# abbomarengo/ml-trainer

Measured on AMD Instinct MI355X. Metric: samples/sec/node, higher is better.
Workload: dtype bf16; 1 GPU; model=src/model.py MLModel (default LeNet-5, 62,006 params), global_batch=32, per_gpu_batch=32, parallelism=dp1, optimizer=sgd lr=1e-3 momentum=0.9, hipgraph_steps=47, graph_prewarm=1, update=in-step, dp_transport=none, loss_finite=True

## Files before the change

ml_trainer_amd/csrc/bindings.cpp:

```cpp
#include <ATen/ATen.h>
#include <c10/hip/HIPStream.h>
#include <pybind11/pybind11.h>
#include <pybind11/stl.h>
#include <torch/extension.h>

#include <cmath>
#include <map>
#include <memory>

#include "mlt_kernels.h"
#include "mlt_comm.h"
#include "mlt_runtime.h"

namespace py = pybind11;
using at::Tensor;

namespace mlt {

hipStream_t cur_stream() { return c10::hip::getCurrentHIPStream().stream(); }

#define CHECK_CUDA_T(t) TORCH_CHECK((t).is_cuda(), #t " must be a device tensor")
#define CHECK_CONTIG(t) TORCH_CHECK((t).is_contiguous(), #t " must be contiguous")
#define CHECK_F32(t) TORCH_CHECK((t).scalar_type() == at::kFloat, #t " must be float32")

// ... 1202 lines not shown
    P_.slab1 = fp("slab1", B * C1 * 640);
    P_.i1 = get("i1", at::kByte, B * C1 * 196).data_ptr<uint8_t>();
    P_.i2 = get("i2", at::kByte, B * FLAT).data_ptr<uint8_t>();
    P_.targets = get("targets", at::kLong, B).data_ptr<int64_t>();
    P_.stats = get("stats", at::kDouble, 2).data_ptr<double>();
    P_.counters = reinterpret_cast<unsigned*>(get("counters", at::kInt, C1 + 1).data_ptr<int32_t>());
    P_.stage = bufs.contains("stage") ? get("stage", at::kByte, B * 3072).data_ptr<uint8_t>() : nullptr;
    P_.stage_meta = bufs.contains("stage_meta") ? get("stage_meta", at::kLong, B * 4).data_ptr<int64_t>() : nullptr;
    if (!P_.stage || !P_.stage_meta) P_.stage = nullptr, P_.stage_meta = nullptr;
    P_.cestat = bufs.contains("cestat") ? get("cestat", at::kDouble, B * 2).data_ptr<double>() : nullptr;
    P_.dtargets = nullptr;
    if (bufs.contains("stage2") && bufs.contains("meta2") && bufs.contains("metaN") && bufs.contains("stepinfo") &&
        bufs.contains("shadow") && bufs.contains("wimg")) {
      P_.stage2 = get("stage2", at::kByte, B * 3072).data_ptr<uint8_t>();
      P_.meta2 = get("meta2", at::kLong, B * 4).data_ptr<int64_t>();
      P_.metaN = get("metaN", at::kLong, B * 4).data_ptr<int64_t>();
      P_.stepinfo = get("stepinfo", at::kLong, 4).data_ptr<int64_t>();
      Tensor sh = bufs["shadow"].cast<Tensor>();
      check_dev(sh, "shadow", at::kShort, 1);
      keep_.push_back(sh);
      P_.shadow = reinterpret_cast<uint16_t*>(sh.data_ptr<int16_t>());
      shadow_n_ = sh.numel();
      P_.wimg = reinterpret_cast<uint16_t*>(get("wimg", at::kShort, lenet_mfma_wimg_elems()).data_ptr<int16_t>());
      TORCH_CHECK(P_.slab1 != nullptr && (int64_t)C1 * 640 >= lenet_mfma_slab_floats(cfg), "slab1 too small");
    }
    if (bufs.contains("trace")) P_.trace = get("trace", at::kFloat, 4096).data_ptr<float>();
    const char* pe = std::getenv("MLT_LENET_PREP");
    if (bufs.contains("prep") && bufs.contains("pmeta") && !(pe && std::string(pe) == "0")) {
      P_.prep = get("prep", at::kByte, B * 8192).data_ptr<uint8_t>();
      P_.pmeta = get("pmeta", at::kLong, B * 4).data_ptr<int64_t>();
    }
    const char* se = std::getenv("MLT_LENET_SPLIT");
    split_ = !(se && std::string(se) == "0");
    A_ = LeNetAug{};
    O_ = LeNetOpt{};
  }

  void set_aug(Tensor data, Tensor perm, Tensor ctrl, Tensor dtargets, int64_t seed, int pad, int flip,
               int batch_stride, std::vector<double> mean, std::vector<double> stdv) {
    A_ = make_aug(data, perm, ctrl, seed, pad, flip, batch_stride, mean, stdv);
    TORCH_CHECK(A_.ctrl != nullptr, "ctrl required");
    check_dev(dtargets, "dtargets", at::kLong, A_.n);
    P_.dtargets = dtargets.data_ptr<int64_t>();
    aug_keep_ = {data, perm, ctrl, dtargets};
    graphs_.clear();
  }

  void clear_aug() {
    A_.data = nullptr;
    P_.dtargets = nullptr;
    graphs_.clear();
  }

  void set_ctrl(Tensor ctrl) {
    check_dev(ctrl, "ctrl", at::kLong, 2, 8);
    A_.ctrl = ctrl.data_ptr<int64_t>();
    ctrl_keep_ = ctrl;
    graphs_.clear();
  }

  void set_opt(Tensor p, Tensor g, c10::optional<Tensor> s1, c10::optional<Tensor> s2, int kind, double lr,
               double momentum, double dampening, double wd, double beta1, double beta2, double eps,
               double lr_decay, double grad_scale, bool nesterov, bool maximize, c10::optional<Tensor> lr_t,
               bool lr_table, std::vector<int64_t> offsets) {
    const int64_t n = p.numel();
    check_dev(p, "p", at::kFloat, n);
// ... 51 lines not shown
    if (comm.is_none()) {
      comm_ = nullptr;
      comm_keep_ = py::none();
    } else {
      comm_ = &comm.cast<PyComm&>().raw();
      comm_keep_ = comm;
    }
    graphs_.clear();
  }

  void set_precision(int p) {
    TORCH_CHECK(p == 0 || p == 1, "precision: 0 (fp32) or 1 (bf16)");
    if (p == 1) TORCH_CHECK(P_.shadow && P_.wimg && P_.stage2 && P_.meta2 && P_.metaN && P_.stepinfo,
                            "bf16 engine buffers missing");
    prec_ = p;
    pack_ver_ = -1;
    graphs_.clear();
  }
  int precision() const { return prec_; }
  void set_fused_dp(bool f) {
    fused_dp_ = f;
    graphs_.clear();
  }
  bool fused_dp() const { return fused_dp_; }
  void set_split(bool s) {
    split_ = s;
    graphs_.clear();
  }
  bool split() const { return split_; }
  bool split_active(int B) const {
    if (prec_ != 1 || B <= 0 || B > max_b_) return false;
    return lenet_mfma_split_active(split_bits(LENET_FWD | LENET_CE | LENET_BWD), B, P_, A_);
  }
  int split_bits(int mode) const {
    return split_ || prec_ != 1 || !(mode & LENET_BWD) ? mode : mode | LENET_NOSPLIT;
  }

  void check_mode(int mode, int B) const {
    TORCH_CHECK(B > 0 && B <= max_b_, "batch ", B, " outside [1, ", max_b_, "]");
    if (prec_ == 1 && (mode & LENET_BWD)) {
      TORCH_CHECK((mode & LENET_FWD) && (mode & LENET_CE), "bf16 engine: training steps are FWD|CE|BWD");
      TORCH_CHECK(A_.ctrl != nullptr && O_.g != nullptr, "bf16 engine: set_ctrl / set_opt first");
      TORCH_CHECK(shadow_n_ >= O_.n, "bf16 engine: shadow smaller than the flat parameters");
    }
    TORCH_CHECK(!((mode & LENET_OPT) && (mode & LENET_REDUCE)),
                "LENET_OPT (fused local update) and LENET_REDUCE (all-reduce + update) are exclusive");
    if (mode & LENET_REDUCE) TORCH_CHECK(A_.ctrl != nullptr, "ctrl required for the data-parallel update");
    if (mode & (LENET_OPT | LENET_REDUCE)) TORCH_CHECK(O_.g != nullptr, "set_opt() first");
    if (mode & LENET_OPT) TORCH_CHECK(A_.ctrl != nullptr, "ctrl required for the fused optimizer");
    if ((mode & LENET_OPT) && O_.lr_table) TORCH_CHECK(A_.ctrl != nullptr, "lr table needs ctrl");
  }

  void run(int mode, int B) {
    check_mode(mode, B);
    const bool mf = prec_ == 1 && (mode & LENET_BWD);
    if (mf) launch_lenet_mfma_pack(cfg_, P_, O_, cur_stream());
    launch_step(cfg_, split_bits(mode), B, P_, A_, O_, comm_, xgmi_, cur_stream(), mf, fused_dp_);
  }

  void reduce_only(int B, bool exchange) {
    TORCH_CHECK(prec_ == 1 && P_.stepinfo && O_.g, "reduce_only: bf16 engine with set_opt");
    TORCH_CHECK(B > 0 && B <= max_b_, "reduce_only: batch");
    if (exchange) {
      TORCH_CHECK(xgmi_ != nullptr, "reduce_only: no xGMI transport");
      const XgmiFused X = xgmi_->fused_view();
      launch_lenet_mfma_reduce(cfg_, B, P_, O_, &X, cur_stream());
    } else {
      launch_lenet_mfma_reduce(cfg_, B, P_, O_, nullptr, cur_stream());
// ... 69 lines not shown
  void replay(int mode, int B, int nsteps) {
    auto it = graphs_.find(key(mode, B, nsteps));
    TORCH_CHECK(it != graphs_.end(), "no captured graph for this (mode, B, nsteps)");
    if (mode & LENET_BWD) sync_shadow();
    it->second->launch(cur_stream());
  }

  size_t graph_nodes(int mode, int B, int nsteps) const {
    auto it = graphs_.find(key(mode, B, nsteps));
    return it == graphs_.end() ? 0 : it->second->num_nodes();
  }

  void reset_graphs() { graphs_.clear(); }

 private:
  static int64_t key(int mode, int B, int nsteps) {
    return ((int64_t)mode << 48) | ((int64_t)B << 16) | (int64_t)nsteps;
  }
  int cfg_;
  int max_b_;
  LeNetPtrs P_{};
  LeNetAug A_{};
  LeNetOpt O_{};
  std::vector<Tensor> keep_, aug_keep_, opt_keep_;
  Tensor ctrl_keep_;
  Communicator* comm_ = nullptr;
  py::object comm_keep_ = py::none();
  XgmiAllReduce* xgmi_ = nullptr;
  py::object xgmi_keep_ = py::none();
  std::map<int64_t, std::unique_ptr<HipGraph>> graphs_;
  int prec_ = 0;
  bool fused_dp_ = true;
  bool split_ = true;
  int64_t shadow_n_ = 0;
  Tensor master_;
  int64_t pack_ver_ = -1;
};

}

PYBIND11_MODULE(TORCH_EXTENSION_NAME, m) {
  using namespace mlt;
  m.doc() = "ml_trainer_amd native gfx950 kernels and runtime";
  m.attr("ARCH") = "gfx950";
  m.def("flat_optim", &flat_optim, py::arg("p"), py::arg("g"), py::arg("s1"), py::arg("s2"), py::arg("kind"),
        py::arg("lr"), py::arg("momentum"), py::arg("dampening"), py::arg("weight_decay"), py::arg("beta1"),
        py::arg("beta2"), py::arg("eps"), py::arg("lr_decay"), py::arg("grad_scale"), py::arg("nesterov"),
        py::arg("maximize"), py::arg("lr_t") = py::none(), py::arg("lr_index") = py::none(),
        py::arg("step_t") = py::none(), py::arg("t_host") = 1.0, py::arg("shadow") = py::none(),
        py::arg("coef") = py::none());
  m.def("optim_chunk_elems", &optim_chunk_elems);
  m.def("flat_optim_seg", &flat_optim_seg, py::arg("p"), py::arg("g"), py::arg("s1"), py::arg("s2"),
        py::arg("chunks"), py::arg("wd"), py::arg("lr"), py::arg("beta1"), py::arg("beta2"), py::arg("eps"),
        py::arg("grad_scale"), py::arg("maximize"), py::arg("lr_t") = py::none(), py::arg("lr_index") = py::none(),
        py::arg("step_t") = py::none(), py::arg("t_host") = 1.0, py::arg("shadow") = py::none(),
        py::arg("coef") = py::none(), py::arg("skip") = py::none(), py::arg("max_blocks") = 0);
  m.def("lamb_step", &lamb_step, py::arg("p"), py::arg("g"), py::arg("m"), py::arg("v"), py::arg("chunks"),
        py::arg("tseg"), py::arg("wd"), py::arg("adapt"), py::arg("part"), py::arg("norms"), py::arg("trust"),
        py::arg("lr"), py::arg("beta1"), py::arg("beta2"), py::arg("eps"), py::arg("grad_scale"),
        py::arg("maximize"), py::arg("lr_t") = py::none(), py::arg("lr_index") = py::none(),
        py::arg("step_t") = py::none(), py::arg("t_host") = 1.0, py::arg("shadow") = py::none(),
        py::arg("coef") = py::none(), py::arg("skip") = py::none(), py::arg("max_blocks") = 0,
        py::arg("stages") = 7);
  m.def("sq_norm", &sq_norm);
  m.def("clip_coef", &clip_coef);
  m.def("cast_bf16", &cast_bf16);
// ... 99 lines not shown
      .def("async_error", &PyComm::async_error)
      .def("abort", &PyComm::abort);
  py::class_<PyXgmi>(m, "XgmiAllReduce", py::dynamic_attr())
      .def(py::init<int64_t, int, int, int, int>(), py::arg("capacity"), py::arg("world"), py::arg("rank"),
           py::arg("device"), py::arg("blocks") = 64)
      .def("handle", &PyXgmi::handle)
      .def("open", &PyXgmi::open)
      .def("all_reduce", &PyXgmi::all_reduce, py::arg("tensor"), py::arg("average") = true)
      .def("error", &PyXgmi::error)
      .def_property_readonly("world", [](PyXgmi& x) { return x.raw().world(); })
      .def_property("timeout_ms", &PyXgmi::timeout_ms, &PyXgmi::set_timeout_ms)
      .def_property("algo", &PyXgmi::algo, &PyXgmi::set_algo)
      .def_property("fault", &PyXgmi::fault, &PyXgmi::set_fault)
      .def_property("fused_two", &PyXgmi::fused_two, &PyXgmi::set_fused_two);
  py::class_<PyPrefetcher>(m, "PinnedPrefetcher")
      .def(py::init<int64_t, int, int>(), py::arg("slot_bytes"), py::arg("depth"), py::arg("device"))
      .def("slot", &PyPrefetcher::slot)
      .def("copy_to_device", &PyPrefetcher::copy_to_device)
      .def("acquire", &PyPrefetcher::acquire)
      .def("release", &PyPrefetcher::release)
      .def("ready", &PyPrefetcher::ready)
      .def("wait", &PyPrefetcher::wait)
      .def_property_readonly("depth", &PyPrefetcher::depth)
      .def_property_readonly("slot_bytes", &PyPrefetcher::slot_bytes);
  py::class_<LeNetEngine>(m, "LeNetEngine")
      .def(py::init<int, int, py::dict>())
      .def("set_aug", &LeNetEngine::set_aug)
      .def("set_comm", &LeNetEngine::set_comm)
      .def("set_xgmi", &LeNetEngine::set_xgmi)
      .def_property("fused_dp", &LeNetEngine::fused_dp, &LeNetEngine::set_fused_dp)
      .def("set_split", &LeNetEngine::set_split)
      .def("split", &LeNetEngine::split)
      .def("split_active", &LeNetEngine::split_active, py::arg("B"))
      .def("clear_aug", &LeNetEngine::clear_aug)
      .def("set_ctrl", &LeNetEngine::set_ctrl)
      .def("set_opt", &LeNetEngine::set_opt)
      .def("set_precision", &LeNetEngine::set_precision)
      .def("precision", &LeNetEngine::precision)
      .def("run", &LeNetEngine::run)
      .def("capture", &LeNetEngine::capture)
      .def("has_graph", &LeNetEngine::has_graph)
      .def("replay", &LeNetEngine::replay)
      .def("invalidate_shadow", &LeNetEngine::invalidate_shadow)
      .def("reduce_only", &LeNetEngine::reduce_only, py::arg("B"), py::arg("exchange"))
      .def("graph_nodes", &LeNetEngine::graph_nodes)
      .def("reset_graphs", &LeNetEngine::reset_graphs);
  m.attr("LENET_FWD") = (int)LENET_FWD;
  m.attr("LENET_CE") = (int)LENET_CE;
  m.attr("LENET_BWD") = (int)LENET_BWD;
  m.attr("LENET_OPT") = (int)LENET_OPT;
  m.attr("LENET_TRACE") = (int)LENET_TRACE;
  m.attr("LENET_REDUCE") = (int)LENET_REDUCE;
}
```

ml_trainer_amd/csrc/include/mlt_kernels.h:

```cpp
#pragma once
#include <hip/hip_runtime.h>
#include <stdint.h>

#include "mlt_optim.h"
#include "mlt_philox.h"

namespace mlt {

void launch_flat_optim(float* p, const float* g, float* s1, float* s2, int64_t n, const OptHyper& h,
                       const float* lr_ptr, const int64_t* lr_index_ptr, const int64_t* step_ptr, float t_host,
                       uint16_t* shadow_bf16, const float* coef_ptr, hipStream_t stream,
                       const unsigned* skip = nullptr);
int optim_chunk_elems();
void launch_flat_optim_seg(float* p, const float* g, float* s1, float* s2, int64_t n, const int* chunks,
                           int nchunks, const float* wd, int nt, const OptHyper& h, const float* lr_ptr,
                           const int64_t* lr_index_ptr, const int64_t* step_ptr, float t_host,
                           uint16_t* shadow_bf16, const float* coef_ptr, const unsigned* skip, int max_blocks,
                           hipStream_t stream);
void launch_lamb_step(float* p, const float* g, float* m, float* v, int64_t n, const int* chunks, int nchunks,
                      const int* tseg, const float* wd, const int* adapt, int nt, float* part, float* norms,
                      float* trust, const OptHyper& h, const float* lr_ptr, const int64_t* lr_index_ptr,
                      const int64_t* step_ptr, float t_host, uint16_t* shadow_bf16, const float* coef_ptr,
                      const unsigned* skip, int max_blocks, int stages, hipStream_t stream);
int sq_norm_partials_needed();
void launch_sq_norm(const float* x, int64_t n, float* part, float* out, hipStream_t stream);
void launch_clip_coef(const float* sq, float max_norm, float* coef, float* total_norm, hipStream_t stream);
void launch_cast_bf16(const float* x, uint16_t* y, int64_t n, hipStream_t stream);
void launch_transpose_bf16(const uint16_t* src, uint16_t* dst, int R, int C, hipStream_t stream);

enum LeNetCfg : int { LENET_DEFAULT = 0, LENET_TINY = 1 };
enum LeNetMode : int {
  LENET_FWD = 1,
  LENET_CE = 2,
  LENET_BWD = 4,
  LENET_OPT = 8,
  LENET_REDUCE = 16,
  LENET_TRACE = 256,
  LENET_STATS_DEFER = 16384,
  LENET_PROBE_NOF1T = 1 << 17,
  LENET_PROBE_NOF1W = 1 << 18,
  LENET_PROBE_NOF2 = 1 << 19,
  LENET_NOSPLIT = 1 << 20,
};

struct LeNetPtrs {
  const float *w1, *b1, *w2, *b2, *w3, *b3, *w4, *b4, *w5, *b5;
  float *gw1, *gb1, *gw2, *gb2, *gw3, *gb3, *gw4, *gb4, *gw5, *gb5;
  float *x, *p1, *p2, *h1, *h2, *logits, *dlogits, *dh2, *dh1, *dflat, *g1, *slab1;
  uint8_t *i1, *i2;
  int64_t* targets;
  const int64_t* dtargets;
  double* stats;
  unsigned* counters;
  uint8_t* stage;
  int64_t* stage_meta;
  double* cestat;
  uint8_t* stage2;
  int64_t* meta2;
  int64_t* metaN;
  int64_t* stepinfo;
  uint16_t* shadow;
  uint16_t* wimg;
  float* trace;
  uint8_t* prep;
  int64_t* pmeta;
};

struct LeNetAug {
  const uint8_t* data;
  int64_t step_host, sie_host;
  const int32_t* perm;
  int64_t* ctrl;
  int64_t n;
  int64_t perm_len;
  uint64_t seed;
  int pad;
  int flip;
  int batch_stride;
  float mean[3], std[3];
  float ascale[3], ashift[3];
};

struct LeNetOpt {
  float *p, *g, *s1, *s2;
  int64_t n;
  OptHyper h;
  const float* lr_ptr;
  int lr_table;
  int64_t off[10];
};

void launch_lenet(int cfg, int mode, int B, const LeNetPtrs& P, const LeNetAug& A, const LeNetOpt& O,
                  hipStream_t stream);
void launch_head_cls_fwd(const float* pooled, int B, int h, const float* wc, const float* bc, int L, float* logits,
                         hipStream_t st);
void launch_head_cls_bwd(const float* dlogits, const float* pooled, const float* wc, int B, int h, int L,
                         uint16_t* dpre, float* dwc, float* dbc, bool accumulate, hipStream_t st);
void launch_lenet_mfma(int cfg, int mode, int B, const LeNetPtrs& P, const LeNetAug& A, const LeNetOpt& O,
                       hipStream_t stream);
bool lenet_mfma_split_active(int mode, int B, const LeNetPtrs& P, const LeNetAug& A);
int lenet_mfma_slab_floats(int cfg);
int lenet_mfma_kw_blocks(int cfg);
void launch_lenet_mfma_apply(int cfg, const LeNetPtrs& P, const LeNetOpt& O, const unsigned* skip, hipStream_t stream);
struct XgmiFused;
void launch_lenet_mfma_dp(int cfg, int mode, int B, const LeNetPtrs& P, const LeNetAug& A, const LeNetOpt& O,
                          const XgmiFused& X, hipStream_t stream);
int lenet_mfma_wimg_elems();
bool lenet_mfma_trace_build();
void launch_lenet_mfma_reduce(int cfg, int B, const LeNetPtrs& P, const LeNetOpt& O, const XgmiFused* X,
                              hipStream_t stream);
int64_t lenet_mfma_xch_granules(int cfg);
void launch_lenet_mfma_pack(int cfg, const LeNetPtrs& P, const LeNetOpt& O, hipStream_t stream);

void launch_cifar_augment(const LeNetAug& A, int B, float* out, int64_t* targets_out, const int64_t* dtargets,
                          hipStream_t stream);

void launch_ce_fwd(const void* logits, bool bf16, const int64_t* tgt, int64_t B, int C, float* dl, float* acc,
                   float* correct, float* loss, int64_t ignore_index, float label_smoothing, hipStream_t st);
void launch_ce_bwd(const float* dl, const float* gout, const float* acc, int64_t n, void* out, bool bf16,
                   hipStream_t st);
void launch_accuracy(const void* logits, bool bf16, const int64_t* tgt, int64_t B, int C, float* out,
                     hipStream_t st);
int loss_partials_needed();
void launch_pointwise_loss_fwd(const float* p, const float* t, int64_t n, int mode, float* g, float* part,
                               float* out, hipStream_t st);
void launch_nll_fwd(const float* logp, const int64_t* tgt, int64_t B, int C, int64_t ignore_index, float* part,
                    float* out, hipStream_t st);
void launch_loss_scale_grad(const float* g, const float* gout, const float* stats, int64_t n, float* out,
                            hipStream_t st);
void launch_nll_bwd(const int64_t* tgt, int64_t B, int C, int64_t ignore_index, const float* gout,
                    const float* stats, float* out, hipStream_t st);
void launch_mcrmse(const float* p, const float* t, int64_t B, int C, float* col, float* out, hipStream_t st);

// ... 129 lines not shown
```

ml_trainer_amd/csrc/kernels/lenet_mfma.hip:

```cpp
#include "lenet_mfma.inc"

namespace mlt {
namespace lm {
void launch_ms(int cfg, int mode, int B, const LeNetPtrs& P, const LeNetAug& A, const LeNetOpt& O, hipStream_t st) {
  if (cfg == LENET_TINY)
    launch_ms_t<DmTiny>(mode, B, P, A, O, st);
  else
    launch_ms_t<DmDefault>(mode, B, P, A, O, st);
}
}

bool lenet_mfma_split_active(int mode, int B, const LeNetPtrs& P, const LeNetAug& A) {
  return lm::split_eligible(mode, B, P, A);
}

void launch_lenet_mfma_reduce(int cfg, int B, const LeNetPtrs& P, const LeNetOpt& O, const XgmiFused* X,
                              hipStream_t stream) {
  if (B <= 0) return;
  if (cfg == LENET_TINY)
    lm::reduce_only<lm::DmTiny>(cfg, B, P, O, X, stream);
  else
    lm::reduce_only<lm::DmDefault>(cfg, B, P, O, X, stream);
}
int lenet_mfma_slab_floats(int cfg) { return cfg == LENET_TINY ? lm::DmTiny::SLABN : lm::DmDefault::SLABN; }
int lenet_mfma_wimg_elems() { return lm::kWimgTot; }
bool lenet_mfma_trace_build() { return lm::kTraceBuild; }
int lenet_mfma_kw_blocks(int cfg) {
  return cfg == LENET_TINY ? lm::mw_conv_blocks<lm::DmTiny>() + lm::mw_fc_blocks<lm::DmTiny>() + 1
                           : lm::mw_conv_blocks<lm::DmDefault>() + lm::mw_fc_blocks<lm::DmDefault>() + 1;
}

void launch_lenet_mfma_apply(int cfg, const LeNetPtrs& P, const LeNetOpt& O, const unsigned* skip, hipStream_t stream) {
  if (O.n <= 0) return;
  const dim3 grid((unsigned)((O.n + 255) / 256));
  if (cfg == LENET_TINY)
    hipLaunchKernelGGL(lm::lenet_mapply<lm::DmTiny>, grid, dim3(256), 0, stream, P, O, skip);
  else
    hipLaunchKernelGGL(lm::lenet_mapply<lm::DmDefault>, grid, dim3(256), 0, stream, P, O, skip);
}

void launch_lenet_mfma_pack(int cfg, const LeNetPtrs& P, const LeNetOpt& O, hipStream_t stream) {
  if (cfg == LENET_TINY)
    lm::pack<lm::DmTiny>(P, O, stream);
  else
    lm::pack<lm::DmDefault>(P, O, stream);
}
// ... 12 lines not shown
```

ml_trainer_amd/csrc/kernels/lenet_mfma.inc:

```
#pragma once
#include <cstdlib>
#include <stdexcept>
#include <type_traits>

#include "mlt_common.h"
#include "mlt_kernels.h"
#include "mlt_optim.h"

namespace mlt {
namespace lm {

typedef __bf16 bf16x8 __attribute__((ext_vector_type(8)));
typedef float f32x4 __attribute__((ext_vector_type(4)));
typedef unsigned u32x4 __attribute__((ext_vector_type(4)));

__device__ __forceinline__ f32x4 mfma(u32x4 a, u32x4 b, f32x4 c) {
  return __builtin_amdgcn_mfma_f32_16x16x32_bf16(__builtin_bit_cast(bf16x8, a), __builtin_bit_cast(bf16x8, b), c, 0,
                                                 0, 0);
}

__device__ __forceinline__ void lbar() { asm volatile("s_waitcnt lgkmcnt(0)\n\ts_barrier" ::: "memory"); }

template <int KW>
__device__ __forceinline__ u32x4 fshift(u32x4 lo, u32x4 hi) {
// ... 48 lines not shown
  }
  if (e < kW2D) {
    const int q = e - kW2F, l = (q >> 3) & 63, j = q & 7, oc = l & 15, tap = 4 * (q >> 9) + (l >> 4);
    return (tap < 25 && oc < C2 && j < C1) ? off_w2 + (oc * C1 + j) * 25 + tap : -1;
  }
  const int q = e - kW2D, l = (q >> 3) & 63, j = q & 7, n = l & 15, gg = l >> 4;
  const int pp = 2 * (q >> 9) + (gg >> 1), oc = 8 * (gg & 1) + j, ic = n >> 1, kh = pp / 6;
  const int kw = pp - 6 * kh - 1 + (n & 1);
  (void)s;
  return (pp < 30 && ic < C1 && oc < C2 && kw >= 0 && kw < 5) ? off_w2 + (oc * C1 + ic) * 25 + kh * 5 + kw : -1;
}

template <int C1_, int C2_, int F1_, int F2_, int NC_>
struct Dm {
  static constexpr int C1 = C1_, C2 = C2_, F1 = F1_, F2 = F2_, NC = NC_, FLAT = C2_ * 25;
  static_assert(C1_ <= 8 && C2_ <= 16 && C2_ % 4 == 0 && F1_ % 4 == 0 && F2_ % 4 == 0 && NC_ <= 64, "dims");
  static constexpr int S1 = C1 * 76, S2OFF = (S1 + 3) & ~3, S2 = C2 * C1 * 25 + C2;
  static constexpr int SLABN = (S2OFF + S2 + 15) & ~15;
};
using DmDefault = Dm<6, 16, 120, 84, 10>;
using DmTiny = Dm<4, 8, 64, 32, 10>;

constexpr int kT = 1024;
constexpr int XCS = 48;
constexpr int P1CS = 32;
constexpr int XHS = 48;
constexpr int P1HS = 24;
constexpr int DCHS = 19;
constexpr int DCCS = 24;
constexpr int D1S = 28 * 32 + 16;
constexpr int kWgT = 256;
constexpr int kP13W = 7;
constexpr int kC1W = 8;
#ifndef MLT_LENET_TRACE_BUILD
#define MLT_LENET_TRACE_BUILD 0
#endif
constexpr bool kTraceBuild = MLT_LENET_TRACE_BUILD != 0;

constexpr int pow2_ge(int v) { return v <= 1 ? 1 : v <= 2 ? 2 : v <= 4 ? 4 : v <= 8 ? 8 : v <= 16 ? 16 : v <= 32 ? 32 : 64; }

template <int KS, int LD, int N, int K>
__device__ __forceinline__ void frag_rows(u32x4 (&f)[KS], const uint16_t* __restrict__ W, int tn) {
  const unsigned lane = threadIdx.x & 63;
  const unsigned row = min(16u * tn + (lane & 15), (unsigned)N - 1);
#pragma unroll
  for (int q = 0; q < KS; ++q) {
    const unsigned col = min(32u * q + 8 * (lane >> 4), (unsigned)((K - 1) / 8 * 8));
    f[q] = ld16(W, row * LD + col);
  }
}
template <int KS>
__device__ __forceinline__ float row_dot(const u32x4 (&f)[KS], const uint16_t* x) {
  const int g = (threadIdx.x & 63) >> 4;
  f32x4 acc = {0.f, 0.f, 0.f, 0.f};
#pragma unroll
  for (int q = 0; q < KS; ++q) acc = mfma(*reinterpret_cast<const u32x4*>(x + 32 * q + 8 * g), f[q], acc);
  return acc[0];
}

typedef short s16x4 __attribute__((ext_vector_type(4)));
typedef __attribute__((address_space(3))) s16x4 lds_s16x4;
template <int FLAT>
__device__ __forceinline__ int f1_chunk(int r, int c) {
  return r * (FLAT / 8 + 1) + (r & 1) + c;
}
template <int F1, int FLAT>
// ... 103 lines not shown
#pragma unroll
  for (int c = 0; c < 3; ++c) {
    const float u = in ? (float)img[(r * 32 + q) * 3 + c] : 0.f;
    v[c] = fmaf(u, A.ascale[c], A.ashift[c]);
  }
}

__device__ __forceinline__ int hmod(uint64_t h, unsigned span) {
  if (span == 9u) return (int)(h % 9u);
  const unsigned hi = (unsigned)(h >> 32) % span, lo = (unsigned)h % span;
  const unsigned r32 = (0xffffffffu % span + 1u) % span;
  return (int)((hi * r32 + lo) % span);
}

__device__ __forceinline__ void aug_params(const LeNetAug& A, int64_t step, int64_t pos, int& ci, int& cj, bool& fl) {
  const uint64_t h = mix64(mix64(A.seed + (uint64_t)step) ^ (uint64_t)pos);
  const unsigned span = 2 * A.pad + 1;
  ci = A.pad ? hmod(h, span) : 0;
  cj = A.pad ? hmod(h >> 20, span) : 0;
  fl = A.flip && ((h >> 40) & 1);
}

__device__ __forceinline__ void pool4(f32x4 a, float bias, float& pv, uint8_t& code) {
  float m = a[0];
  int k = 0;
  if (a[1] > m) { m = a[1]; k = 1; }
  if (a[2] > m) { m = a[2]; k = 2; }
  if (a[3] > m) { m = a[3]; k = 3; }
  m += bias;
  pv = m > 0.f ? m : 0.f;
  code = m > 0.f ? (uint8_t)k : (uint8_t)4;
}

template <class D, bool SPLIT>
__global__ __launch_bounds__(kT) void lenet_ms(uint8_t* __restrict__ pstage2, int64_t* __restrict__ pmeta2,
                                               const int64_t* __restrict__ pctrl, const uint16_t* __restrict__ pwimg,
                                               int64_t* __restrict__ pmetaN, int mode, float inv_B, LeNetPtrs P,
                                               LeNetAug A, LeNetOpt O, int B) {
  constexpr int C1 = D::C1, C2 = D::C2, FLAT = D::FLAT, F1 = D::F1, F2 = D::F2, NC = D::NC;
  using S = KsLds<D>;
  static_assert(offsetof(typename S::V::Fw, w2f) == offsetof(typename S::V::Fw, w1f) + 2 * kW2F,
                "forward fragment images must be contiguous");
  static_assert(sizeof(S) <= 160 * 1024, "LDS");
  __shared__ S L;
  const int bi = (int)blockIdx.x;
  const bool roleW = SPLIT && bi >= B;
  const bool doW = !SPLIT || roleW, doD = !SPLIT || !roleW;
  const int b = roleW ? bi - B : bi, t = threadIdx.x, lane = t & 63, g = lane >> 4, m = lane & 15;
  const int w = __builtin_amdgcn_readfirstlane(t >> 6);
  auto stamp = [&](int k) {
    if constexpr (!kTraceBuild) return;
    if (!(mode & LENET_TRACE)) return;
    lbar();
    __builtin_amdgcn_sched_barrier(0);
    unsigned long long c, wc;
    asm volatile("s_memtime %0\n\ts_memrealtime %1\n\ts_waitcnt lgkmcnt(0)" : "=s"(c), "=s"(wc)::"memory");
    __builtin_amdgcn_sched_barrier(0);
    if (t == 0) {
      L.tr[k] = c;
      if (k == 0) L.tr[14] = wc;
      if (k == 13) L.tr[15] = wc;
    }
  };
  if (kTraceBuild && (mode & LENET_TRACE) && t < 32) L.tr[t] = 0ull;
  if (kTraceBuild && (mode & LENET_TRACE) && t < 96) (&L.wtr[0][0])[t] = 0ull;
  auto wstamp = [&](int k) {
    if constexpr (!kTraceBuild) return;
    if (!(mode & LENET_TRACE)) return;
    __builtin_amdgcn_sched_barrier(0);
    unsigned long long c;
    asm volatile("s_waitcnt lgkmcnt(0)\n\ts_memtime %0\n\ts_waitcnt lgkmcnt(0)" : "=s"(c)::"memory");
    __builtin_amdgcn_sched_barrier(0);
    if (lane == 0) L.wtr[k][w] = c;
  };
  stamp(0);
  unsigned long long tb0 = 0;
  if (kTraceBuild && (mode & LENET_TRACE)) tb0 = __builtin_amdgcn_s_memrealtime();

  const bool aug = A.data != nullptr;
  const bool pre_on = aug && P.pmeta != nullptr && P.prep != nullptr;
  using F1M = typename S::F;
// ... 498 lines not shown
        }
      };
      switch (tt >> 1) {
        case 0: tile(std::integral_constant<int, 0>{}); break;
        case 1: tile(std::integral_constant<int, 1>{}); break;
        case 2: tile(std::integral_constant<int, 2>{}); break;
        case 3: tile(std::integral_constant<int, 3>{}); break;
        default: tile(std::integral_constant<int, 4>{}); break;
      }
    }
  };
  auto block_clock = [&]() {
    if constexpr (!kTraceBuild) return;
    if (!((mode & LENET_TRACE) && P.trace && bi < 200)) return;
    lbar();
    if (t == 0) {
      reinterpret_cast<unsigned long long*>(P.trace)[600 + 2 * bi] = tb0;
      reinterpret_cast<unsigned long long*>(P.trace)[601 + 2 * bi] = __builtin_amdgcn_s_memrealtime();
    }
  };
  auto p11_end = [&]() __attribute__((always_inline)) {
    wstamp(3);
    lbar();
    stamp(7);
  };
  auto c1w_row = [&](int slot, int yy, u32x4& lo, u32x4& hi) __attribute__((always_inline)) {
    const int c = m / 5, kh = m - 5 * c;
    const bool valid = m < 15;
    const uint16_t* xrow = L.xc + ((valid ? c : 0) * 32 + (valid ? kh : 0)) * XCS + 8 * g;
    const int Y = (28 / kP13W) * slot + yy;
    lo = *reinterpret_cast<const u32x4*>(xrow + Y * XCS);
    hi = *reinterpret_cast<const u32x4*>(xrow + Y * XCS + 8);
  };
  auto c1w = [&](int slot, auto PREc, const u32x4* plo, const u32x4* phi) __attribute__((always_inline)) {
    constexpr bool PRE = decltype(PREc)::value;
    const bool valid = m < 15;
    const int x0 = 8 * g;
    const uint16_t* drow = L.v.k.d1 + min(m, C1 - 1) * D1S + x0;
    constexpr u32x4 ONES = {0x3F803F80u, 0x3F803F80u, 0x3F803F80u, 0x3F803F80u};
    const u32x4 Z = {0u, 0u, 0u, 0u};
    f32x4 acc[5];
#pragma unroll
    for (int k = 0; k < 5; ++k) acc[k] = f32x4{0.f, 0.f, 0.f, 0.f};
#pragma unroll
    for (int yy = 0; yy < 28 / kP13W; ++yy) {
      const int Y = (28 / kP13W) * slot + yy;
      u32x4 bq = *reinterpret_cast<const u32x4*>(drow + Y * 32);
      if (m >= C1) bq = Z;
      u32x4 lo, hi;
      if constexpr (PRE) {
        lo = plo[yy];
        hi = phi[yy];
      } else {
        c1w_row(slot, yy, lo, hi);
      }
      acc[0] = mfma(valid ? fshift<0>(lo, hi) : (m == 15 ? ONES : Z), bq, acc[0]);
      acc[1] = mfma(valid ? fshift<1>(lo, hi) : Z, bq, acc[1]);
      acc[2] = mfma(valid ? fshift<2>(lo, hi) : Z, bq, acc[2]);
      acc[3] = mfma(valid ? fshift<3>(lo, hi) : Z, bq, acc[3]);
      acc[4] = mfma(valid ? fshift<4>(lo, hi) : Z, bq, acc[4]);
    }
#pragma unroll
    for (int kw = 0; kw < 5; ++kw)
#pragma unroll
      for (int r = 0; r < 4; ++r) L.u.b.scr[((slot * 5 + kw) * 16 + 4 * g + r) * 16 + m] = acc[kw][r];
  };
  if constexpr (SPLIT) {
    if (roleW) {
      if (w >= 6) wgrad_tile(w - 6);
      wstamp(3);
      block_clock();
      return;
    }
    lbar();
    stamp(6);
    if (w < 7) {
      dgrad();
      p11_end();
    } else if (w < 7 + kP13W) {
      u32x4 xlo[28 / kP13W], xhi[28 / kP13W];
#pragma unroll
      for (int yy = 0; yy < 28 / kP13W; ++yy) c1w_row(w - 7, yy, xlo[yy], xhi[yy]);
      p11_end();
      c1w(w - 7, std::true_type{}, xlo, xhi);
    } else {
      p11_end();
    }
  } else {
    lbar();
    stamp(6);
    if (w < 7) {
      dgrad();
    } else {
      const int t0 = w - 7, t1 = w == 7 ? 2 : w - 6;
      for (int tt0 = t0; tt0 < t1; ++tt0) wgrad_tile(w == 7 && tt0 == 1 ? 9 : tt0);
    }
    p11_end();
    if (w < kP13W) c1w(w, std::false_type{}, nullptr, nullptr);
  }
  wstamp(4);
  lbar();
  stamp(23);
  for (int e = t; e < 5 * 256; e += kT) {
    const int kw = e >> 8, i = (e >> 4) & 15, oc = e & 15;
    float v = L.u.b.scr[e];
#pragma unroll
    for (int p = 1; p < kP13W; ++p) v += L.u.b.scr[p * 1280 + e];
    if (oc < C1) {
      if (i < 15) slab[oc * 76 + (i / 5) * 25 + (i % 5) * 5 + kw] = v;
      else if (kw == 0) slab[oc * 76 + 75] = v;
    }
  }
  stamp(24);
  stamp(13);
  if (kTraceBuild && (mode & LENET_TRACE) && b == 0 && t < 32 && P.trace) reinterpret_cast<unsigned long long*>(P.trace)[t] = L.tr[t];
  if (kTraceBuild && (mode & LENET_TRACE) && b == 0 && t < 96 && P.trace)
    reinterpret_cast<unsigned long long*>(P.trace)[1024 + t] = (&L.wtr[0][0])[t];
  block_clock();
}

struct Ctx {
  bool on;
  float lr, t;
};


constexpr int kXchTwo = 16;
template <int XT>
struct Xch {
  static constexpr int WT = XT & (kXchTwo - 1);
  static constexpr bool TWO = (XT & kXchTwo) != 0;
  static_assert(!TWO || WT > 1, "two-phase exchange: two ranks or more");
  static constexpr bool on = WT > 0;
  uint64_t* gr[WT > 0 ? WT : 1];
  uint64_t* mine;
  uint64_t* rd[WT > 0 ? WT : 1];
  uint64_t* rmine;
  unsigned* err;
  unsigned* derr;
  long long timeout;
  int rank;
  unsigned tag;
  bool dead;
  bool withhold;
  bool corrupt;
  float scale;

  __device__ __forceinline__ void st(int64_t i, float v) const {
    const unsigned u = __float_as_uint(v) ^ (corrupt ? 1u : 0u);
// ... 639 lines not shown
  }
}

template <class D>
void pack(const LeNetPtrs& P, const LeNetOpt& O, hipStream_t st) {
  const int64_t tot = O.n > kWimgTot ? O.n : kWimgTot;
  hipLaunchKernelGGL(lenet_mpack<D>, dim3((unsigned)((tot + 255) / 256)), dim3(256), 0, st, O.p, O.n, P.shadow, P.wimg,
                     O.off[0], O.off[2], O.off[4], O.off[6], O.off[8]);
}

static int probe_bits() {
  static const int v = [] {
    const char* e = std::getenv("MLT_LENET_PROBE");
    return e ? std::atoi(e) & (LENET_PROBE_NOF1T | LENET_PROBE_NOF1W | LENET_PROBE_NOF2) : 0;
  }();
  return v;
}

inline int nprep(const LeNetPtrs& P, const LeNetAug& A, int B) {
  return (A.data && A.perm && P.prep && P.pmeta && P.dtargets && P.stepinfo && P.stage2 && P.meta2) ? B : 0;
}

inline int device_cus() {
  static int cus[64] = {};
  int dev = 0;
  if (hipGetDevice(&dev) != hipSuccess || dev < 0 || dev >= 64) return 0;
  if (cus[dev] == 0) {
    int n = 0;
    cus[dev] = hipDeviceGetAttribute(&n, hipDeviceAttributeMultiprocessorCount, dev) == hipSuccess && n > 0 ? n : -1;
  }
  return cus[dev] > 0 ? cus[dev] : 0;
}

inline bool split_eligible(int mode, int B, const LeNetPtrs& P, const LeNetAug& A) {
  if (!(mode & LENET_BWD) || (mode & LENET_NOSPLIT)) return false;
  if (A.data && !(P.prep && P.pmeta)) return false;
  return B > 0 && 2 * B <= device_cus();
}

template <class D>
void launch_ms_t(int mode, int B, const LeNetPtrs& P, const LeNetAug& A, const LeNetOpt& O, hipStream_t st) {
  const float inv_B = 1.f / (float)B;
  if (split_eligible(mode, B, P, A))
    hipLaunchKernelGGL((lenet_ms<D, true>), dim3(2 * B), dim3(kT), 0, st, P.stage2, P.meta2, A.ctrl, P.wimg, P.metaN,
                       mode, inv_B, P, A, O, B);
  else
    hipLaunchKernelGGL((lenet_ms<D, false>), dim3(B), dim3(kT), 0, st, P.stage2, P.meta2, A.ctrl, P.wimg, P.metaN,
                       mode, inv_B, P, A, O, B);
}

template <class D>
void run(int mode, int B, const LeNetPtrs& P, const LeNetAug& A, const LeNetOpt& O, hipStream_t st) {
  mode |= probe_bits();
  launch_ms_t<D>(mode, B, P, A, O, st);
  const int nblk = mw_conv_blocks<D>() + mw_fc_blocks<D>() + 1;
  hipLaunchKernelGGL(lenet_mw<D>, dim3(nblk + nprep(P, A, B)), dim3(kWgT), 0, st, P.slab1, P.p2, P.dh1, P.h1, P.dh2,
                     mode, B, P, O, A.ctrl, A);
}

void launch_ms(int cfg, int mode, int B, const LeNetPtrs& P, const LeNetAug& A, const LeNetOpt& O, hipStream_t st);

template <class D>
void run_dp(int cfg, int mode, int B, const LeNetPtrs& P, const LeNetAug& A, const LeNetOpt& O, const XgmiFused& X,
            hipStream_t st) {
  const int nblk = mw_conv_blocks<D>() + mw_fc_blocks<D>() + 1;
  if (X.G < nblk) throw std::runtime_error("lenet dp step: transport block counters < reduction blocks");
  if (X.cap < xch_granules<D>()) throw std::runtime_error("lenet dp step: transport granule region too small");
  mode |= probe_bits();
  launch_ms(cfg, mode, B, P, A, O, st);
  launch_mwx_any(cfg, dim3(nblk + nprep(P, A, B)), st, P, mode | LENET_OPT, B, O, A.ctrl, A, X);
}

template <class D>
void reduce_only(int cfg, int B, const LeNetPtrs& P, const LeNetOpt& O, const XgmiFused* X, hipStream_t st) {
  const int nblk = mw_conv_blocks<D>() + mw_fc_blocks<D>() + 1;
  const int m = LENET_FWD | LENET_CE | LENET_BWD;
  if (!X) {
    hipLaunchKernelGGL(lenet_mw<D>, dim3(nblk), dim3(kWgT), 0, st, P.slab1, P.p2, P.dh1, P.h1, P.dh2, m, B, P, O,
                       (int64_t*)nullptr, LeNetAug{});
    return;
  }
// ... 7 lines not shown
```

ml_trainer_amd/models/lenet_engine.py:

```python
from __future__ import annotations

import math
from typing import Optional, Sequence

import torch

from ml_trainer_amd.models.lenet import MLModel, lenet_buffers, _param_names
from ml_trainer_amd.ops._ext import require_native
from ml_trainer_amd.utils.flat import FlatParams

CIFAR_MEAN = (0.4914, 0.4822, 0.4465)
CIFAR_STD = (0.2023, 0.1994, 0.2010)


def fused_dp_enabled() -> bool:
    import os
    return os.environ.get("MLT_LENET_FUSED_DP", "1") != "0"


def fused_dp_forced() -> bool:
    import os
    return os.environ.get("MLT_LENET_FUSED_DP", "1") == "2"


# ... 273 lines not shown

    def start_epoch(self, indices: torch.Tensor, lr_values: Optional[Sequence[float]] = None) -> None:
        n = indices.numel()
        if n > self.perm.numel():
            raise ValueError("epoch permutation larger than perm capacity")
        self.perm[:n].copy_(indices.to(torch.int32), non_blocking=True)
        self.ctrl[1:2].zero_()
        self._reset_staging()
        if lr_values is not None:
            if not self._use_table:
                raise RuntimeError("engine not configured with an lr table")
            vals = torch.tensor(list(lr_values), dtype=torch.float32)
            self.lr_table[:vals.numel()].copy_(vals, non_blocking=False)
        elif self.optimizer is not None:
            self.optimizer.lr_tensor(0)

    def _reset_staging(self) -> None:
        for k in ("stage_meta", "meta2", "metaN", "pmeta"):
            self.bufs[k].fill_(-1)

    def reset_stats(self) -> None:
        self.stats.zero_()

    def read_stats(self, n_batches: int):
        s = self.stats.cpu().tolist()
        return s[0] / max(n_batches, 1), s[1] / max(n_batches, 1)

    def set_split(self, on: bool) -> None:
        self.eng.set_split(bool(on))

    def split_active(self, B: int) -> bool:
        return bool(self.eng.split_active(int(B)))

    @property
    def fused(self) -> bool:
        return self.world_size == 1 and self.dp_transport == "none"

    def use_transport(self, comm=None, xgmi=None, fused: Optional[bool] = None) -> None:
        if (comm is None) == (xgmi is None):
            raise ValueError("pass exactly one of comm / xgmi")
        self.comm, self.xgmi = comm, xgmi
        if comm is not None:
            self.eng.set_xgmi(None)
            self.eng.set_comm(comm)
            self.dp_transport = "rccl"
        else:
            if fused is None:
                fused = fused_dp_enabled()
            fused = bool(fused) and self.precision == "bf16"
            self.eng.set_comm(None)
            self.eng.set_xgmi(xgmi)
            self.eng.fused_dp = fused
            self.fused_two = fused and bool(getattr(xgmi, "fused_two", False))
            if fused:
                self.dp_transport = "xgmi-fused"
            else:
                self.dp_transport = "xgmi-twoshot" if getattr(xgmi, "algo", 0) == 1 else "xgmi-oneshot"

    @property
    def in_graph_collective(self) -> bool:
        return self.dp_transport in ("rccl", "xgmi-oneshot", "xgmi-twoshot", "xgmi-fused")

    def _train_mode(self) -> int:
        C = self.C
        base = C.LENET_FWD | C.LENET_CE | C.LENET_BWD
        if self.fused:
# ... 146 lines not shown
```

Measured before the change: 2.154 million samples/s.

## Split conv1 weight-gradient role across three blocks per sample by kernel column

```diff
diff --git a/ml_trainer_amd/csrc/bindings.cpp b/ml_trainer_amd/csrc/bindings.cpp
--- a/ml_trainer_amd/csrc/bindings.cpp
+++ b/ml_trainer_amd/csrc/bindings.cpp
@@ -1258,6 +1258,13 @@
     }
     const char* se = std::getenv("MLT_LENET_SPLIT");
     split_ = !(se && std::string(se) == "0");
+    const char* sd = std::getenv("MLT_LENET_SPLIT_D");
+    split_parts_ = 0;
+    if (sd && *sd) {
+      const int n = std::atoi(sd);
+      TORCH_CHECK(lenet_mfma_split_parts_valid(n), "MLT_LENET_SPLIT_D=", sd, ": not a built part count");
+      split_parts_ = n;
+    }
     A_ = LeNetAug{};
     O_ = LeNetOpt{};
   }
@@ -1375,8 +1382,19 @@
     if (prec_ != 1 || B <= 0 || B > max_b_) return false;
     return lenet_mfma_split_active(split_bits(LENET_FWD | LENET_CE | LENET_BWD), B, P_, A_);
   }
+  void set_split_parts(int n) {
+    TORCH_CHECK(lenet_mfma_split_parts_valid(n), "set_split_parts: ", n, " is not a built part count");
+    split_parts_ = n;
+    graphs_.clear();
+  }
+  int split_parts() const { return split_parts_; }
+  int split_blocks(int B) const {
+    if (prec_ != 1 || B <= 0 || B > max_b_) return 1;
+    return lenet_mfma_split_blocks(split_bits(LENET_FWD | LENET_CE | LENET_BWD), B, P_, A_);
+  }
   int split_bits(int mode) const {
-    return split_ || prec_ != 1 || !(mode & LENET_BWD) ? mode : mode | LENET_NOSPLIT;
+    if (prec_ != 1 || !(mode & LENET_BWD)) return mode;
+    return split_ ? mode | (split_parts_ << LENET_SPLITD_SHIFT) : mode | LENET_NOSPLIT;
   }
 
   void check_mode(int mode, int B) const {
@@ -1512,6 +1530,7 @@
   int prec_ = 0;
   bool fused_dp_ = true;
   bool split_ = true;
+  int split_parts_ = 0;
   int64_t shadow_n_ = 0;
   Tensor master_;
   int64_t pack_ver_ = -1;
@@ -1677,6 +1696,9 @@
       .def("set_split", &LeNetEngine::set_split)
       .def("split", &LeNetEngine::split)
       .def("split_active", &LeNetEngine::split_active, py::arg("B"))
+      .def("set_split_parts", &LeNetEngine::set_split_parts, py::arg("n"))
+      .def("split_parts", &LeNetEngine::split_parts)
+      .def("split_blocks", &LeNetEngine::split_blocks, py::arg("B"))
       .def("clear_aug", &LeNetEngine::clear_aug)
       .def("set_ctrl", &LeNetEngine::set_ctrl)
       .def("set_opt", &LeNetEngine::set_opt)
diff --git a/ml_trainer_amd/csrc/include/mlt_kernels.h b/ml_trainer_amd/csrc/include/mlt_kernels.h
--- a/ml_trainer_amd/csrc/include/mlt_kernels.h
+++ b/ml_trainer_amd/csrc/include/mlt_kernels.h
@@ -41,6 +41,8 @@
   LENET_PROBE_NOF1W = 1 << 18,
   LENET_PROBE_NOF2 = 1 << 19,
   LENET_NOSPLIT = 1 << 20,
+  LENET_SPLITD_SHIFT = 21,
+  LENET_SPLITD_MASK = 7 << 21,
 };
 
 struct LeNetPtrs {
@@ -99,6 +101,8 @@
 void launch_lenet_mfma(int cfg, int mode, int B, const LeNetPtrs& P, const LeNetAug& A, const LeNetOpt& O,
                        hipStream_t stream);
 bool lenet_mfma_split_active(int mode, int B, const LeNetPtrs& P, const LeNetAug& A);
+int lenet_mfma_split_blocks(int mode, int B, const LeNetPtrs& P, const LeNetAug& A);
+bool lenet_mfma_split_parts_valid(int n);
 int lenet_mfma_slab_floats(int cfg);
 int lenet_mfma_kw_blocks(int cfg);
 void launch_lenet_mfma_apply(int cfg, const LeNetPtrs& P, const LeNetOpt& O, const unsigned* skip, hipStream_t stream);
diff --git a/ml_trainer_amd/csrc/kernels/lenet_mfma.hip b/ml_trainer_amd/csrc/kernels/lenet_mfma.hip
--- a/ml_trainer_amd/csrc/kernels/lenet_mfma.hip
+++ b/ml_trainer_amd/csrc/kernels/lenet_mfma.hip
@@ -11,7 +11,16 @@
 }
 
 bool lenet_mfma_split_active(int mode, int B, const LeNetPtrs& P, const LeNetAug& A) {
+  return lm::split_eligible(mode, B, P, A) > 1;
+}
+int lenet_mfma_split_blocks(int mode, int B, const LeNetPtrs& P, const LeNetAug& A) {
   return lm::split_eligible(mode, B, P, A);
+}
+bool lenet_mfma_split_parts_valid(int n) {
+  if (n == 0) return true;
+  for (int nd : lm::kSplitND)
+    if (n == nd) return true;
+  return false;
 }
 
 void launch_lenet_mfma_reduce(int cfg, int B, const LeNetPtrs& P, const LeNetOpt& O, const XgmiFused* X,
diff --git a/ml_trainer_amd/csrc/kernels/lenet_mfma.inc b/ml_trainer_amd/csrc/kernels/lenet_mfma.inc
--- a/ml_trainer_amd/csrc/kernels/lenet_mfma.inc
+++ b/ml_trainer_amd/csrc/kernels/lenet_mfma.inc
@@ -104,6 +104,10 @@
 constexpr int kWgT = 256;
 constexpr int kP13W = 7;
 constexpr int kC1W = 8;
+constexpr int kSplitND[] = {1, 3};
+constexpr int kSplitAuto = 3;
+constexpr int c1w_kw_lo(int nd, int d) { return nd == 3 ? 2 * d : 0; }
+constexpr int c1w_kw_hi(int nd, int d) { return nd == 3 ? (d == 2 ? 5 : 2 * d + 2) : 5; }
 #ifndef MLT_LENET_TRACE_BUILD
 #define MLT_LENET_TRACE_BUILD 0
 #endif
@@ -273,7 +277,7 @@
   code = m > 0.f ? (uint8_t)k : (uint8_t)4;
 }
 
-template <class D, bool SPLIT>
+template <class D, int ND>
 __global__ __launch_bounds__(kT) void lenet_ms(uint8_t* __restrict__ pstage2, int64_t* __restrict__ pmeta2,
                                                const int64_t* __restrict__ pctrl, const uint16_t* __restrict__ pwimg,
                                                int64_t* __restrict__ pmetaN, int mode, float inv_B, LeNetPtrs P,
@@ -284,10 +288,22 @@
                 "forward fragment images must be contiguous");
   static_assert(sizeof(S) <= 160 * 1024, "LDS");
   __shared__ S L;
+  constexpr bool SPLIT = ND > 0;
   const int bi = (int)blockIdx.x;
-  const bool roleW = SPLIT && bi >= B;
+  int pd = 0, b = bi;
+  if constexpr (ND > 1) {
+#pragma unroll
+    for (int k = 1; k <= ND; ++k) {
+      if (bi >= k * B) {
+        pd = k;
+        b = bi - k * B;
+      }
+    }
+  }
+  const bool roleW = ND > 1 ? pd == ND : SPLIT && bi >= B;
+  if constexpr (ND == 1) b = roleW ? bi - B : bi;
   const bool doW = !SPLIT || roleW, doD = !SPLIT || !roleW;
-  const int b = roleW ? bi - B : bi, t = threadIdx.x, lane = t & 63, g = lane >> 4, m = lane & 15;
+  const int t = threadIdx.x, lane = t & 63, g = lane >> 4, m = lane & 15;
   const int w = __builtin_amdgcn_readfirstlane(t >> 6);
   auto stamp = [&](int k) {
     if constexpr (!kTraceBuild) return;
@@ -852,8 +868,11 @@
     lo = *reinterpret_cast<const u32x4*>(xrow + Y * XCS);
     hi = *reinterpret_cast<const u32x4*>(xrow + Y * XCS + 8);
   };
-  auto c1w = [&](int slot, auto PREc, const u32x4* plo, const u32x4* phi) __attribute__((always_inline)) {
+  auto c1w = [&](int slot, auto PREc, auto K0c, auto K1c, const u32x4* plo, const u32x4* phi)
+                 __attribute__((always_inline)) {
     constexpr bool PRE = decltype(PREc)::value;
+    constexpr int K0 = decltype(K0c)::value, K1 = decltype(K1c)::value;
+    static_assert(0 <= K0 && K0 < K1 && K1 <= 5, "kw range");
     const bool valid = m < 15;
     const int x0 = 8 * g;
     const uint16_t* drow = L.v.k.d1 + min(m, C1 - 1) * D1S + x0;
@@ -874,16 +893,33 @@
       } else {
         c1w_row(slot, yy, lo, hi);
       }
-      acc[0] = mfma(valid ? fshift<0>(lo, hi) : (m == 15 ? ONES : Z), bq, acc[0]);
-      acc[1] = mfma(valid ? fshift<1>(lo, hi) : Z, bq, acc[1]);
-      acc[2] = mfma(valid ? fshift<2>(lo, hi) : Z, bq, acc[2]);
-      acc[3] = mfma(valid ? fshift<3>(lo, hi) : Z, bq, acc[3]);
-      acc[4] = mfma(valid ? fshift<4>(lo, hi) : Z, bq, acc[4]);
-    }
-#pragma unroll
-    for (int kw = 0; kw < 5; ++kw)
+      if constexpr (K0 <= 0 && 0 < K1) acc[0] = mfma(valid ? fshift<0>(lo, hi) : (m == 15 ? ONES : Z), bq, acc[0]);
+      if constexpr (K0 <= 1 && 1 < K1) acc[1] = mfma(valid ? fshift<1>(lo, hi) : Z, bq, acc[1]);
+      if constexpr (K0 <= 2 && 2 < K1) acc[2] = mfma(valid ? fshift<2>(lo, hi) : Z, bq, acc[2]);
+      if constexpr (K0 <= 3 && 3 < K1) acc[3] = mfma(valid ? fshift<3>(lo, hi) : Z, bq, acc[3]);
+      if constexpr (K0 <= 4 && 4 < K1) acc[4] = mfma(valid ? fshift<4>(lo, hi) : Z, bq, acc[4]);
+    }
+#pragma unroll
+    for (int kw = K0; kw < K1; ++kw)
 #pragma unroll
       for (int r = 0; r < 4; ++r) L.u.b.scr[((slot * 5 + kw) * 16 + 4 * g + r) * 16 + m] = acc[kw][r];
+  };
+  auto c1w_part = [&](int slot, const u32x4* plo, const u32x4* phi) __attribute__((always_inline)) {
+    auto part = [&](auto Dc) __attribute__((always_inline)) {
+      constexpr int d = decltype(Dc)::value;
+      c1w(slot, std::true_type{}, std::integral_constant<int, c1w_kw_lo(ND, d)>{},
+          std::integral_constant<int, c1w_kw_hi(ND, d)>{}, plo, phi);
+    };
+    if constexpr (ND <= 1) {
+      part(std::integral_constant<int, 0>{});
+    } else {
+      static_assert(ND == 3, "role-D parts: 1 or 3");
+      switch (pd) {
+        case 0: part(std::integral_constant<int, 0>{}); break;
+        case 1: part(std::integral_constant<int, 1>{}); break;
+        default: part(std::integral_constant<int, 2>{}); break;
+      }
+    }
   };
   if constexpr (SPLIT) {
     if (roleW) {
@@ -902,7 +938,7 @@
 #pragma unroll
       for (int yy = 0; yy < 28 / kP13W; ++yy) c1w_row(w - 7, yy, xlo[yy], xhi[yy]);
       p11_end();
-      c1w(w - 7, std::true_type{}, xlo, xhi);
+      c1w_part(w - 7, xlo, xhi);
     } else {
       p11_end();
     }
@@ -916,12 +952,23 @@
       for (int tt0 = t0; tt0 < t1; ++tt0) wgrad_tile(w == 7 && tt0 == 1 ? 9 : tt0);
     }
     p11_end();
-    if (w < kP13W) c1w(w, std::false_type{}, nullptr, nullptr);
+    if (w < kP13W)
+      c1w(w, std::false_type{}, std::integral_constant<int, 0>{}, std::integral_constant<int, 5>{}, nullptr, nullptr);
   }
   wstamp(4);
   lbar();
   stamp(23);
-  for (int e = t; e < 5 * 256; e += kT) {
+  int e0 = 0, e1 = 5 * 256;
+  if constexpr (ND > 1) {
+#pragma unroll
+    for (int k = 0; k < ND; ++k) {
+      if (pd == k) {
+        e0 = c1w_kw_lo(ND, k) * 256;
+        e1 = c1w_kw_hi(ND, k) * 256;
+      }
+    }
+  }
+  for (int e = e0 + t; e < e1; e += kT) {
     const int kw = e >> 8, i = (e >> 4) & 15, oc = e & 15;
     float v = L.u.b.scr[e];
 #pragma unroll
@@ -933,8 +980,8 @@
   }
   stamp(24);
   stamp(13);
-  if (kTraceBuild && (mode & LENET_TRACE) && b == 0 && t < 32 && P.trace) reinterpret_cast<unsigned long long*>(P.trace)[t] = L.tr[t];
-  if (kTraceBuild && (mode & LENET_TRACE) && b == 0 && t < 96 && P.trace)
+  if (kTraceBuild && (mode & LENET_TRACE) && bi == 0 && t < 32 && P.trace) reinterpret_cast<unsigned long long*>(P.trace)[t] = L.tr[t];
+  if (kTraceBuild && (mode & LENET_TRACE) && bi == 0 && t < 96 && P.trace)
     reinterpret_cast<unsigned long long*>(P.trace)[1024 + t] = (&L.wtr[0][0])[t];
   block_clock();
 }
@@ -1640,21 +1687,33 @@
   return cus[dev] > 0 ? cus[dev] : 0;
 }
 
-inline bool split_eligible(int mode, int B, const LeNetPtrs& P, const LeNetAug& A) {
-  if (!(mode & LENET_BWD) || (mode & LENET_NOSPLIT)) return false;
-  if (A.data && !(P.prep && P.pmeta)) return false;
-  return B > 0 && 2 * B <= device_cus();
+inline int split_eligible(int mode, int B, const LeNetPtrs& P, const LeNetAug& A) {
+  if (!(mode & LENET_BWD) || (mode & LENET_NOSPLIT)) return 1;
+  if (A.data && !(P.prep && P.pmeta)) return 1;
+  if (B <= 0) return 1;
+  int want = (mode & LENET_SPLITD_MASK) >> LENET_SPLITD_SHIFT;
+  if (want == 0) want = kSplitAuto;
+  const int cus = device_cus();
+  int nd = 0;
+  for (int k : kSplitND)
+    if (k <= want && (k + 1) * B <= cus) nd = k;
+  return nd + 1;
+}
+
+template <class D, int ND>
+void launch_ms_nd(int mode, int B, const LeNetPtrs& P, const LeNetAug& A, const LeNetOpt& O, hipStream_t st) {
+  hipLaunchKernelGGL((lenet_ms<D, ND>), dim3((ND + 1) * B), dim3(kT), 0, st, P.stage2, P.meta2, A.ctrl, P.wimg,
+                     P.metaN, mode, 1.f / (float)B, P, A, O, B);
 }
 
 template <class D>
 void launch_ms_t(int mode, int B, const LeNetPtrs& P, const LeNetAug& A, const LeNetOpt& O, hipStream_t st) {
-  const float inv_B = 1.f / (float)B;
-  if (split_eligible(mode, B, P, A))
-    hipLaunchKernelGGL((lenet_ms<D, true>), dim3(2 * B), dim3(kT), 0, st, P.stage2, P.meta2, A.ctrl, P.wimg, P.metaN,
-                       mode, inv_B, P, A, O, B);
-  else
-    hipLaunchKernelGGL((lenet_ms<D, false>), dim3(B), dim3(kT), 0, st, P.stage2, P.meta2, A.ctrl, P.wimg, P.metaN,
-                       mode, inv_B, P, A, O, B);
+  switch (split_eligible(mode, B, P, A) - 1) {
+    case 0: launch_ms_nd<D, 0>(mode, B, P, A, O, st); break;
+    case 1: launch_ms_nd<D, 1>(mode, B, P, A, O, st); break;
+    case 3: launch_ms_nd<D, 3>(mode, B, P, A, O, st); break;
+    default: throw std::runtime_error("lenet_ms: role-D part count not built");
+  }
 }
 
 template <class D>
diff --git a/ml_trainer_amd/models/lenet_engine.py b/ml_trainer_amd/models/lenet_engine.py
--- a/ml_trainer_amd/models/lenet_engine.py
+++ b/ml_trainer_amd/models/lenet_engine.py
@@ -329,6 +329,12 @@
     def split_active(self, B: int) -> bool:
         return bool(self.eng.split_active(int(B)))
 
+    def set_split_parts(self, n: int) -> None:
+        self.eng.set_split_parts(int(n))
+
+    def split_blocks(self, B: int) -> int:
+        return int(self.eng.split_blocks(int(B)))
+
     @property
     def fused(self) -> bool:
         return self.world_size == 1 and self.dp_transport == "none"
```

Measured after the change: 2.206 million samples/s (median of 6 runs). +2.4%, better.
